# NVIDIA/DALI

Hardware: NVIDIA H100
Metric: images/sec decode+resize+CMN (batch 256, 1080p JPEG) (higher is better)
Workload: dtype u8

## Files before the change

### dali_b200/csrc/jpeg.cu

```cuda
#include "common.cuh"
#include <algorithm>
#include <cstring>
#include <map>
#include <thread>

namespace dalib200 {

constexpr int kDcLutBits = 9, kAcLutBits = 11;
constexpr int kDcLutSize = 1 << kDcLutBits, kAcLutSize = 1 << kAcLutBits;
constexpr int kLutWords = 2 * kDcLutSize + 2 * kAcLutSize;
constexpr int kSyncThreads = 256;
constexpr int kChunkBytes = 4096;
constexpr int kMaxBlocksPerMcu = 10;
constexpr int kMaxLog2Sub = 10;

constexpr int kLongLut = 512;
struct HuffSlow {
  int32_t maxcode[18];
  int32_t valoff[18];
  uint8_t vals[256];
  int32_t long_base, long_n;
  uint16_t long_lut[kLongLut];
};

struct TableSet {
  uint32_t lut[kLutWords];
  uint16_t lut16[kLutWords];
  HuffSlow slow[4];
};
__host__ __device__ inline int LutOffset(int t) { return t < 2 ? t * kDcLutSize : 2 * kDcLutSize + (t - 2) * kAcLutSize; }

struct QuantSet { uint16_t q[4][64]; };

enum JpegColor : int32_t {
  kColorGray = 0,
// ... 193 lines not shown
#pragma unroll
      for (int w = 0; w < 8; w++) { if (w < (int)wid) woff += wsum[w][r]; tot += wsum[w][r]; }
      uint32_t pos = head + total + (uint32_t)(woff + incl[r] - cw.nk[r]);
      const uint32_t i = (uint32_t)r * 1024u + threadIdx.x * 4u;
#pragma unroll
      for (int k = 0; k < 4; k++)
        if (i + k < len && !((cw.dm[r] >> (8 * k)) & 1u)) ob[pos++] = (uint8_t)(cw.w[r] >> (8 * k));
      total += (uint32_t)tot;
    }
    __syncthreads();
    const uint32_t nwords = (head + total + 3u) >> 2, tailb = (head + total) & 3u;
    uint32_t *cw32 = reinterpret_cast<uint32_t *>(clean) + (out_base >> 2);
    for (uint32_t wd = threadIdx.x; wd < nwords; wd += blockDim.x) {
      const uint32_t v = obuf[wd];
      const bool full = (wd > 0 || head == 0) && (wd + 1 < nwords || tailb == 0);
      if (full) {
        cw32[wd] = __byte_perm(v, 0u, 0x0123);
      } else {
        const uint32_t lo = wd == 0 ? head : 0u, hi = (wd + 1 == nwords && tailb) ? tailb : 4u;
        for (uint32_t b = lo; b < hi; b++) reinterpret_cast<uint8_t *>(cw32 + wd)[3u - b] = (uint8_t)(v >> (8 * b));
      }
    }
    if (c0 + kChunkBytes >= u.raw_len) {
      const uint32_t e0 = out_base + total, e1 = u.clean_off + ((u.raw_len + 32u + 15u) & ~15u);
      for (uint32_t q = e0 + threadIdx.x; q < e1; q += blockDim.x) clean[(q & ~3u) | (3u - (q & 3u))] = 0;
    }
    __syncthreads();
  }
}

struct SmemSrc {
  uint32_t base; int lsw;
  __device__ __forceinline__ uint32_t load(uint32_t g) const { return lds_u32(base + ((g ^ ((g >> lsw) & 31u)) << 2)); }
};
struct SmemLut { uint32_t base; __device__ __forceinline__ uint32_t load(uint32_t i) const { return lds_u32(base + (i << 2)); } };
struct GlobalLut { const uint32_t *p; __device__ __forceinline__ uint32_t load(uint32_t i) const { return __ldg(p + i); } };
template <int STRIDE> struct SmemTbl { uint32_t base; __device__ __forceinline__ uint32_t load(int c) const { return lds_u32(base + (uint32_t)c * (STRIDE * 4u)); } };
struct GlobalSrc {
  const uint32_t *w;
  __device__ __forceinline__ uint32_t load(uint32_t g) const { return __ldg(w + g); }
};

template <class Src>
struct BitWindow {
  uint32_t hi, lo, g;
  int avail;
  __device__ __forceinline__ void init(const Src &s, uint32_t word, uint32_t sh) {
    const uint32_t w0 = s.load(word), w1 = s.load(word + 1);
    hi = __funnelshift_l(w1, w0, sh);
    lo = w1 << sh;
    avail = 64 - (int)sh;
    g = word + 2;
  }
  __device__ __forceinline__ void consume(const Src &s, uint32_t e) {
    hi = __funnelshift_l(lo, hi, e);
    lo = __funnelshift_l(0u, lo, e);
    avail -= (int)(e & 31u);
    const uint32_t w = s.load(g);
    const bool need = avail < 32;
    const uint32_t a = (uint32_t)avail & 31u;
    hi |= (need ? w : 0u) >> a;
    lo = need ? (w << ((32u - a) & 31u)) : lo;
    avail += need ? 32 : 0;
    g += need ? 1u : 0u;
  }
};

constexpr uint64_t kStateMask = (1ull << 42) - 1;
constexpr uint32_t kMaxChainLen = 4095;
__device__ __forceinline__ uint64_t pack_state(uint32_t p, int c, int z, uint32_t cnt = 0, uint32_t t = 0) {
  return (uint64_t)p | ((uint64_t)(uint32_t)c << 32) | ((uint64_t)(uint32_t)z << 36) | ((uint64_t)min(cnt, 1023u) << 42) | ((uint64_t)t << 52);
}
__device__ __forceinline__ uint32_t state_count(uint64_t s) { return (uint32_t)(s >> 42) & 1023u; }

__device__ __forceinline__ uint32_t make_entry(uint32_t len, uint32_t sym, bool is_dc) {
  const uint32_t s = sym & 15u, r = sym >> 4;
  const uint32_t adv = is_dc ? 1u : (s == 0 ? (r == 15u ? 16u : 64u) : r + 1u);
  return (len + s) | (s << 8) | (len << 12) | (adv << 20);
}

__device__ __forceinline__ uint32_t make_entry16(uint32_t len, uint32_t sym, bool is_dc) {
  const uint32_t s = sym & 15u, r = sym >> 4;
  const uint32_t adv = is_dc ? 1u : (s == 0 ? (r == 15u ? 16u : 64u) : r + 1u);
  return (len + s) | (s << 5) | (adv << 9);
}

__device__ __noinline__ uint32_t slow_lookup(const HuffSlow *__restrict__ slow, uint32_t toff, uint32_t hi, bool is_dc) {
  const int tbl = toff < 2u * kDcLutSize ? (int)(toff / kDcLutSize) : 2 + (int)((toff - 2u * kDcLutSize) / kAcLutSize);
  const HuffSlow *sl = slow + tbl;
  const int32_t code16 = (int32_t)(hi >> 16);
  if (sl->long_n > 0) {
    const int idx = min(max(code16 - sl->long_base, 0), sl->long_n - 1);
    const uint32_t e = sl->long_lut[idx];
    return e ? e : 16u;
  }
  uint32_t len = (is_dc ? kDcLutBits : kAcLutBits) + 1;
  while (len <= 16 && code16 >= sl->maxcode[len]) len++;
  uint32_t sym = 0;
  if (len > 16) len = 16;
  else sym = sl->vals[(sl->valoff[len] + (code16 >> (16 - len))) & 0xFF];
  return len | (sym << 8);
}
__device__ __forceinline__ uint32_t slow_symbol(const HuffSlow *__restrict__ slow, uint32_t toff, uint32_t hi, bool is_dc) {
  const uint32_t ls = slow_lookup(slow, toff, hi, is_dc);
  return make_entry(ls & 0xFFu, ls >> 8, is_dc);
}
__device__ __forceinline__ uint32_t slow_symbol16(const HuffSlow *__restrict__ slow, uint32_t toff, uint32_t hi, bool is_dc) {
  const uint32_t ls = slow_lookup(slow, toff, hi, is_dc);
  return make_entry16(ls & 0xFFu, ls >> 8, is_dc);
}

template <class Src, class Lut, class Tbl>
__device__ __forceinline__ void decode_span(const Src &src, BitWindow<Src> &win, const Lut &lut, const HuffSlow *__restrict__ slow,
                                            const Tbl &tbl, int bpm, uint32_t &pos, uint32_t end, int &c, int &z, uint32_t &nb) {
  uint32_t tb12 = tbl.load(c);
  while (pos < end) {
    const uint32_t e_ac = lut.load((tb12 >> 16) + (win.hi >> (32 - kAcLutBits)));
    const bool is_dc = z == 0;
    uint32_t e = e_ac;
    if (is_dc) e = lut.load((tb12 & 0xFFFFu) + (win.hi >> (32 - kDcLutBits)));
    if (__builtin_expect(e == 0, 0)) e = slow_symbol(slow, is_dc ? (tb12 & 0xFFFFu) : (tb12 >> 16), win.hi, is_dc);
    const uint32_t tb = e & 31u, adv = e >> 20;
    win.consume(src, e);
    pos += tb;
    z += (int)adv;
    const bool endb = z >= 64;
    const int c1 = c + 1 == bpm ? 0 : c + 1;
    nb += endb ? 1u : 0u;
    c = endb ? c1 : c;
    z = endb ? 0 : z;
    if (endb) tb12 = tbl.load(c);
  }
}

__device__ __forceinline__ int find_unit_by_subseq(const JpegUnit *u, int ub, int ue, int j) {
  int lo = ub, hi = ue - 1;
  while (lo < hi) {
    int mid = (lo + hi + 1) >> 1;
    if (u[mid].first_subseq <= j) lo = mid; else hi = mid - 1;
  }
  return lo;
}

struct HuffCtx {
  const JpegImage *images; int nimages;
  const int32_t *block_image;
// ... 99 lines not shown
}

__device__ __forceinline__ void push_chain(const HuffCtx &cx, int list, uint32_t pos, int c, int z, uint32_t t, int64_t g, int img) {
  const uint32_t k = atomicAdd(&cx.chain_count[list], 1u);
  cx.chains[list][k] = make_uint4(pos, (uint32_t)c | ((uint32_t)z << 8) | (t << 16), (uint32_t)g, (uint32_t)img);
}

__global__ void __launch_bounds__(kSyncThreads) huff_sync_intra_kernel(HuffCtx cx) {
  extern __shared__ __align__(16) uint32_t hsm[];
  const SyncSmem sm = carve_sync_smem(hsm, cx.log2_sub);
  const int img_i = cx.block_image[blockIdx.x];
  const JpegImage &im = cx.images[img_i];
  const SubGeom sg = sync_block_prologue(cx, im, sm);
  const HuffSlow *slow = sm.slow;
  const int lsw = cx.log2_sub - 5;
  const SmemSrc src{smem_u32(sm.sw), lsw};
  const SmemLut lut{smem_u32(sm.lut)};
  const SmemTbl<1> tbl{smem_u32(sm.tbl)};
  BitWindow<SmemSrc> win;
  uint32_t pos = sg.jl << cx.log2_sub, nb = 0;
  int c = 0, z = 0;
  if (sg.valid) {
    win.init(src, (uint32_t)threadIdx.x << lsw, 0);
    decode_span(src, win, lut, slow, tbl, im.bpm, pos, sm.col_end[threadIdx.x], c, z, nb);
    sm.exitst[threadIdx.x] = pack_state(pos, c, z);
    sm.cnt[threadIdx.x] = nb;
  }
  __syncthreads();
  if (sm.col_cont[threadIdx.x]) {
    if (threadIdx.x + 1 == kSyncThreads) {
      push_chain(cx, 0, pos, c, z, 1u, sg.g + 1, img_i);
    } else {
      const uint32_t x = threadIdx.x + 1;
      nb = 0;
      decode_span(src, win, lut, slow, tbl, im.bpm, pos, sm.col_end[x], c, z, nb);
      const uint64_t ns = pack_state(pos, c, z);
      const bool same = sm.exitst[x] == ns;
      sm.exitst[x] = ns; sm.cnt[x] = nb;
      if (!same && sm.col_cont[x]) push_chain(cx, 0, pos, c, z, 2u, sg.g + 2, img_i);
    }
  }
  __syncthreads();
  if (sg.valid) {
    const uint32_t t = threadIdx.x > 0 && sm.col_cont[threadIdx.x - 1] ? 1u : 0u;
    cx.s_state[sg.g] = sm.exitst[threadIdx.x] | ((uint64_t)min(sm.cnt[threadIdx.x], 1023u) << 42) | ((uint64_t)t << 52);
  }
}

constexpr int kTailThreads = 256;
constexpr int kTailColWords = 36;
struct ColSrc {
  uint32_t base;
  __device__ __forceinline__ uint32_t load(uint32_t g) const { return lds_u32(base + g * (kTailThreads * 4u)); }
};

__device__ __forceinline__ void walk_chain(const HuffCtx &cx, const uint4 rec, int out_list, int max_visits, const uint32_t *s_lut,
                                           const HuffSlow *s_slow, int s_table_set, uint32_t *col, uint32_t *tblcol) {
  const int img_i = (int)rec.w;
  const JpegImage &im = cx.images[img_i];
  int64_t g = rec.z;
  const int j = (int)(g - im.subseq_begin);
  const int ui = im.unit_end - im.unit_begin == 1 ? im.unit_begin : find_unit_by_subseq(cx.units, im.unit_begin, im.unit_end, j);
  const JpegUnit &u = cx.units[ui];
  const uint32_t clean_bits = cx.unit_clean_len[ui] * 8u;
  const uint32_t nsub_eff = (clean_bits + (1u << cx.log2_sub) - 1) >> cx.log2_sub;
  uint32_t jl = (uint32_t)(j - u.first_subseq);
#pragma unroll
  for (int b = 0; b < kMaxBlocksPerMcu; b++) tblcol[b * kTailThreads] = tbl_word(im, b);
  const bool shared_tables = im.table_set == s_table_set;
  uint32_t pos = rec.x, t = rec.y >> 16;
  int c = (int)(rec.y & 0xFF), z = (int)((rec.y >> 8) & 0xFF);
  const int sub_words = 1 << (cx.log2_sub - 5);
  for (int visit = 0;;) {
    uint32_t nb = 0;
    const uint32_t end = min((jl + 1) << cx.log2_sub, clean_bits);
    if (shared_tables && sub_words + 4 <= kTailColWords) {
      const uint4 *p4 = reinterpret_cast<const uint4 *>(cx.clean + u.clean_off + ((size_t)jl << (cx.log2_sub - 3)));
      for (int q = 0; q < sub_words / 4 + 1; q++) {
        const uint4 v = __ldg(p4 + q);
        col[(4 * q + 0) * kTailThreads] = v.x; col[(4 * q + 1) * kTailThreads] = v.y;
        col[(4 * q + 2) * kTailThreads] = v.z; col[(4 * q + 3) * kTailThreads] = v.w;
      }
      const ColSrc src{smem_u32(col)};
      const uint32_t rel = pos - (jl << cx.log2_sub);
      BitWindow<ColSrc> win;
      win.init(src, rel >> 5, rel & 31u);
      decode_span(src, win, SmemLut{smem_u32(s_lut)}, s_slow, SmemTbl<kTailThreads>{smem_u32(tblcol)}, im.bpm, pos, end, c, z, nb);
    } else {
      const GlobalSrc src{reinterpret_cast<const uint32_t *>(cx.clean + u.clean_off)};
      BitWindow<GlobalSrc> win;
      win.init(src, pos >> 5, pos & 31u);
      decode_span(src, win, GlobalLut{cx.tables[im.table_set].lut}, cx.tables[im.table_set].slow, SmemTbl<kTailThreads>{smem_u32(tblcol)},
                  im.bpm, pos, end, c, z, nb);
    }
    const uint64_t ns = pack_state(pos, c, z, nb, t);
    const uint64_t old = atomicMax(reinterpret_cast<unsigned long long *>(cx.s_state + g), (unsigned long long)ns);
    if ((uint32_t)(old >> 52) >= t) break;
    if (((old ^ ns) & kStateMask) == 0) break;
    if (jl + 1 >= nsub_eff || t >= kMaxChainLen) break;
    g++; jl++; t++;
    if (++visit >= max_visits) { push_chain(cx, out_list, pos, c, z, t, g, img_i); break; }
  }
}

__global__ void __launch_bounds__(kTailThreads) huff_sync_walk_kernel(HuffCtx cx, int in_list, int out_list, int max_visits) {
  extern __shared__ __align__(16) uint32_t tsm[];
  const uint32_t n = cx.chain_count[in_list];
  if (blockIdx.x * blockDim.x >= n) return;
  uint32_t *s_lut = tsm;
  HuffSlow *s_slow = reinterpret_cast<HuffSlow *>(s_lut + kLutWords);
  uint32_t *col = reinterpret_cast<uint32_t *>(s_slow + 4) + threadIdx.x;
  uint32_t *tblcol = reinterpret_cast<uint32_t *>(s_slow + 4) + kTailColWords * kTailThreads + threadIdx.x;
  const int s_table_set = cx.images[0].table_set;
  {
    const uint4 *src = reinterpret_cast<const uint4 *>(cx.tables[s_table_set].lut);
// ... 23 lines not shown
    __syncthreads();
    for (uint32_t base = 0; base < nsub_eff; base += blockDim.x) {
      const uint32_t i = base + threadIdx.x;
      const uint32_t v = i < nsub_eff ? state_count(cx.s_state[g0 + i]) : 0u;
      uint32_t incl = v;
      for (int o = 1; o < 32; o <<= 1) { uint32_t x = __shfl_up_sync(0xffffffffu, incl, o); if ((threadIdx.x & 31) >= o) incl += x; }
      if ((threadIdx.x & 31) == 31) warp_tot[threadIdx.x >> 5] = incl;
      __syncthreads();
      uint32_t woff = 0, tot = 0;
      for (int w = 0; w < (int)(blockDim.x >> 5); w++) { if (w < (int)(threadIdx.x >> 5)) woff += warp_tot[w]; tot += warp_tot[w]; }
      if (i < nsub_eff) cx.s_n[g0 + i] = carry + woff + incl - v;
      __syncthreads();
      if (threadIdx.x == 0) carry += tot;
      __syncthreads();
    }
    if (threadIdx.x == 0) {
      if ((int64_t)carry * 64 < u.nslots) cx.status[blockIdx.x] = 1;
      cx.unit_nblk[ui] = (uint32_t)min((int64_t)carry, u.nslots >> 6);
    }
  }
}

constexpr int kWriteThreads = 384;
struct WriteSmem {
  uint16_t *lut; uint32_t *sw, *tbl, *blkbuf; uint8_t *zig; HuffSlow *slow; const uint8_t **colptr;
};
__host__ __device__ inline size_t write_sw_words(int log2_sub) { return (size_t)(kWriteThreads + look_ahead_cols(log2_sub)) << (log2_sub - 5); }
__host__ __device__ inline size_t write_smem_bytes(int log2_sub) {
  return kLutWords * 2 + write_sw_words(log2_sub) * 4 + 16 * 4  + 64  + (size_t)kWriteThreads * 128;
}
__device__ __forceinline__ WriteSmem carve_write_smem(uint32_t *base, int log2_sub) {
  WriteSmem s;
  s.lut = reinterpret_cast<uint16_t *>(base);
  s.sw = base + kLutWords / 2;
  s.tbl = s.sw + write_sw_words(log2_sub);
  s.zig = reinterpret_cast<uint8_t *>(s.tbl + 16);
  s.slow = nullptr;
  s.blkbuf = reinterpret_cast<uint32_t *>(s.zig + 64);
  s.colptr = reinterpret_cast<const uint8_t **>(s.blkbuf);
  return s;
}

__global__ void __launch_bounds__(kWriteThreads) huff_write_kernel(HuffCtx cx) {
  extern __shared__ __align__(16) uint32_t hsm[];
  const WriteSmem sm = carve_write_smem(hsm, cx.log2_sub);
  const JpegImage &im = cx.images[cx.wblock_image[blockIdx.x]];
  const int lsw = cx.log2_sub - 5;
  {
    const uint4 *src = reinterpret_cast<const uint4 *>(cx.tables[im.table_set].lut16);
    uint4 *dst = reinterpret_cast<uint4 *>(sm.lut);
    for (int i = threadIdx.x; i < kLutWords * 2 / 16; i += blockDim.x) dst[i] = __ldg(src + i);
    if (threadIdx.x < kMaxBlocksPerMcu) sm.tbl[threadIdx.x] = tbl_word(im, threadIdx.x);
    if (threadIdx.x < 64) sm.zig[threadIdx.x] = c_zigzag[threadIdx.x];
  }
  SubGeom sg;
  {
    const int j = (blockIdx.x - im.wblock_begin) * kWriteThreads + threadIdx.x;
    sg.valid = j < im.nsub;
    sg.ui = 0; sg.jl = 0; sg.nsub_eff = 0; sg.clean_bits = 0;
    sg.g = (int64_t)im.subseq_begin + j;
    const uint8_t *ptr = nullptr;
    if (sg.valid) {
      sg.ui = im.unit_end - im.unit_begin == 1 ? im.unit_begin : find_unit_by_subseq(cx.units, im.unit_begin, im.unit_end, j);
      const JpegUnit &u = cx.units[sg.ui];
      sg.clean_bits = cx.unit_clean_len[sg.ui] * 8u;
      sg.nsub_eff = (sg.clean_bits + (1u << cx.log2_sub) - 1) >> cx.log2_sub;
      sg.jl = (uint32_t)(j - u.first_subseq);
      sg.valid = sg.jl < sg.nsub_eff;
      if (sg.valid) ptr = cx.clean + u.clean_off + ((size_t)sg.jl << (cx.log2_sub - 3));
    }
    sm.colptr[threadIdx.x] = ptr;
    const int la_cols = look_ahead_cols(cx.log2_sub);
    if (threadIdx.x == kWriteThreads - 1)
      for (int q = 1; q <= la_cols; q++) sm.colptr[kWriteThreads - 1 + q] = ptr ? ptr + ((size_t)q << (cx.log2_sub - 3)) : nullptr;
    __syncthreads();
    const int cpc = 1 << (cx.log2_sub - 7);
    for (int ch = threadIdx.x; ch < (kWriteThreads + la_cols) * cpc; ch += blockDim.x) {
      const int col = ch / cpc, o = ch - col * cpc;
      const uint8_t *p = sm.colptr[col];
      if (p) {
        const uint4 v = __ldg(reinterpret_cast<const uint4 *>(p) + o);
        const uint32_t g = ((uint32_t)col << lsw) + 4u * o, x = (uint32_t)col & 31u;
        sm.sw[(g + 0) ^ x] = v.x; sm.sw[(g + 1) ^ x] = v.y; sm.sw[(g + 2) ^ x] = v.z; sm.sw[(g + 3) ^ x] = v.w;
      }
    }
    __syncthreads();
  }
  const HuffSlow *slow = cx.tables[im.table_set].slow;
  const SmemSrc src{smem_u32(sm.sw), lsw};
  const uint32_t lane = threadIdx.x & 31u;
  const uint32_t a_lut = smem_u32(sm.lut), a_tbl = smem_u32(sm.tbl), a_zig = smem_u32(sm.zig);
  const uint32_t a_wbuf = smem_u32(sm.blkbuf) + (threadIdx.x & ~31u) * 128u;
  const uint32_t a_mybuf = a_wbuf + lane * 128u;
#pragma unroll
  for (int j = 0; j < 32; j++) sts_u32(a_mybuf + 4u * j, 0u);
  __syncwarp();
  uint32_t pos = 0, nb = 0, end = 0, hard_end = 0, blk0 = 0, blk_limit = 0;
  int c = 0, z = 0;
  bool active = sg.valid;
  if (active) {
    const JpegUnit &u = cx.units[sg.ui];
    if (sg.jl > 0) {
      const uint64_t prev = cx.s_state[sg.g - 1];
      pos = (uint32_t)prev; c = (int)((prev >> 32) & 15u); z = (int)((prev >> 36) & 63u);
    }
    end = min((sg.jl + 1) << cx.log2_sub, sg.clean_bits);
    hard_end = sg.clean_bits;
    const uint32_t ublk = (uint32_t)(u.slot_base >> 6);
    blk0 = ublk + cx.s_n[sg.g];
    blk_limit = ublk + (uint32_t)(u.nslots >> 6);
    active = pos < end && blk0 < blk_limit;
  }
  bool own = z == 0;
  BitWindow<SmemSrc> win;
  {
    const uint32_t rel = active ? pos - (sg.jl << cx.log2_sub) : 0u;
    win.init(src, ((uint32_t)threadIdx.x << lsw) + (rel >> 5), rel & 31u);
  }
  int16_t *coef = cx.coef + im.coef_off;
  int16_t *dcv = cx.dc + im.coef_off / 64;
  const int bpm = im.bpm;
  uint32_t tb12 = lds_u32(a_tbl + 4u * c);
  while (__any_sync(0xffffffffu, active)) {
    bool flush = false;
    const uint32_t blk = blk0 + nb;
    if (active) {
      const uint32_t e_ac = lds_u16(a_lut + 2u * ((tb12 >> 16) + (win.hi >> (32 - kAcLutBits))));
      const bool is_dc = z == 0;
      uint32_t e = e_ac;
      if (is_dc) e = lds_u16(a_lut + 2u * ((tb12 & 0xFFFFu) + (win.hi >> (32 - kDcLutBits))));
      if (__builtin_expect(e == 0, 0)) e = slow_symbol16(slow, is_dc ? (tb12 & 0xFFFFu) : (tb12 >> 16), win.hi, is_dc);
      const uint32_t tb = e & 31u, adv = e >> 9, s = (e >> 5) & 15u;
      {
        const uint32_t len = tb - s;
        const uint32_t bits = (uint32_t)(((uint64_t)(win.hi << len)) >> (32u - s));
        const int v = (int)bits - ((s == 0 || ((bits >> (s - 1u)) & 1u)) ? 0 : (int)((1u << s) - 1u));
        if (own) {
          if (is_dc) {
            dcv[blk] = (int16_t)v;
          } else if (s) {
            const uint32_t nat = lds_u8(a_zig + min((uint32_t)z + adv - 1u, 63u));
            sts_u16(a_mybuf + 4u * ((nat >> 1) ^ lane) + 2u * (nat & 1u), (uint32_t)v);
          }
        }
      }
      win.consume(src, e);
      pos += tb;
      z += (int)adv;
      const bool endb = z >= 64;
      const int c1 = c + 1 == bpm ? 0 : c + 1;
      flush = endb && own;
      nb += endb ? 1u : 0u;
      own = own || endb;
      c = endb ? c1 : c;
      z = endb ? 0 : z;
      if (endb) tb12 = lds_u32(a_tbl + 4u * c);
      active = blk0 + nb < blk_limit && (pos < end || (z != 0 && pos < hard_end));
    }
    uint32_t m = __ballot_sync(0xffffffffu, flush);
    while (m) {
      const uint32_t L = __ffs(m) - 1u;
      m &= m - 1u;
      const uint32_t fb = __shfl_sync(0xffffffffu, blk, L);
      const uint32_t a_src = a_wbuf + L * 128u + 4u * (lane ^ L);
      const uint32_t w = lds_u32(a_src);
      sts_u32(a_src, 0u);
      reinterpret_cast<uint32_t *>(coef + (size_t)fb * 64)[lane] = w;
    }
    __syncwarp();
// ... 826 lines not shown
  std::vector<int> post_sample;
  std::vector<size_t> post_off;
  std::vector<int32_t> out_shape;
  std::vector<uint8_t> planes_only;
  std::vector<JpegGeo> geo;
  std::vector<int64_t> first_work;
  std::vector<int64_t> first_fused;
  int64_t total_work = 0, total_fused = 0, total_post_px = 0;
  size_t post_bytes = 0;
  uint8_t *d_post = nullptr; size_t d_post_cap = 0;
  JpegPost *d_posts = nullptr; size_t d_posts_cap = 0;
  std::vector<ParsedJpeg> parsed;
  std::vector<JpegImage> images;
  std::vector<JpegUnit> units;
  std::vector<TableSet> tables;
  std::vector<QuantSet> quants;
  std::vector<int64_t> first_quad, first_item;
  std::vector<int32_t> block_image;
  std::vector<int32_t> wblock_image;
  std::vector<const uint8_t *> src_ptr;
  bool source_stable = false;
  int last_upload_direct = 0;
  std::vector<size_t> stage_off;
  size_t raw_bytes = 0, clean_bytes = 0;
  uint32_t nchunks = 0;
  int64_t total_subseq = 0, total_coefs = 0, total_plane_bytes = 0, total_quads = 0, total_items = 0;
  int total_blocks_sync = 0, total_blocks_write = 0;
  int log2_sub = 10;
  uint8_t *h_stage = nullptr; size_t h_stage_cap = 0;
  uint8_t *d_stage = nullptr; size_t d_stage_cap = 0;
  size_t desc_bytes = 0, off_images = 0, off_units = 0, off_tables = 0, off_quants = 0, off_quads = 0, off_items = 0, off_work = 0, off_fused = 0, off_blkimg = 0, off_wblkimg = 0, off_raw = 0;
  uint8_t *d_clean = nullptr; size_t d_clean_cap = 0;
  uint32_t *d_chunk = nullptr; size_t d_chunk_cap = 0;
  uint32_t *d_unit_len = nullptr; size_t d_unit_cap = 0;
  uint64_t *d_state = nullptr; uint32_t *d_n = nullptr; size_t d_sub_cap = 0;
  uint4 *d_chain1 = nullptr, *d_chain2 = nullptr, *d_chain3 = nullptr;
  size_t d_chain1_cap = 0, d_chain2_cap = 0, d_chain3_cap = 0;
  uint32_t *d_chain_count = nullptr; size_t d_chain_count_cap = 0;
  int walk_max_grid = 0;
  int16_t *d_coef = nullptr; size_t d_coef_cap = 0;
  int16_t *d_dc = nullptr; size_t d_dc_cap = 0;
  uint8_t *d_planes = nullptr; size_t d_planes_cap = 0;
  int32_t *d_status = nullptr; size_t d_status_cap = 0;
  uint32_t *d_unit_nblk = nullptr; size_t d_unit_nblk_cap = 0;
  int32_t *h_status = nullptr; size_t h_status_cap = 0;
  cudaEvent_t uploaded = nullptr, img_uploaded = nullptr;
  uint8_t *h_images = nullptr; size_t h_images_cap = 0;
// ... 176 lines not shown
  p->dtype = prm->dtype; p->adjust_orientation = prm->adjust_orientation != 0;
  p->posts.clear(); p->post_sample.clear(); p->post_off.clear();
  p->out_shape.assign((size_t)3 * n, 0);
  p->planes_only.assign(n, 0);
  p->geo.assign(n, JpegGeo());
  p->first_work.assign(n, 0);
  p->first_fused.assign(n, 0);

  p->parsed.assign(n, ParsedJpeg());
  p->images.assign(n, JpegImage());
  p->units.clear(); p->tables.clear(); p->quants.clear(); p->src_ptr.clear(); p->block_image.clear(); p->wblock_image.clear();
  p->first_quad.assign(n, 0);
  p->first_item.assign(n, 0);
  p->prog_images.clear(); p->prog_scans.clear(); p->prog_huff.clear(); p->prog_wave_begin.clear(); p->prog_first_blk.clear();
  p->prog_total_blocks = 0;
  std::map<std::string, int> table_cache, quant_cache, prog_table_cache;
  size_t raw = 0, clean = 0;
  uint32_t chunks = 0;
  int64_t subseq = 0, coefs = 0, planes = 0;
  int sync_blocks = 0, write_blocks = 0;
  size_t total_len = 0;
  for (int i = 0; i < n; i++) total_len += lengths[i];
  int log2_bytes = kMaxLog2Sub - 3;
  if (const char *ev = getenv("DALIB200_JPEG_SUBSEQ_BYTES")) { int v = atoi(ev); log2_bytes = v >= 256 ? 8 : v >= 128 ? 7 : v >= 64 ? 6 : 5; }
  while (log2_bytes > 5 && (total_len >> log2_bytes) < 200000) log2_bytes--;
  p->log2_sub = log2_bytes + 3;
  const size_t sub_bytes = (size_t)1 << log2_bytes;
  for (int i = 0; i < n; i++) {
    ParsedJpeg &j = p->parsed[i];
    DB_CHECK_ARG(streams[i] && lengths[i] > 0, "decoders.image: sample %d is empty", i);
    int rc = ParseHeaders(streams[i], lengths[i], j, true);
    if (rc) { std::string m = dalib200GetLastError(); SetLastError("decoders.image: sample %d: %s", i, m.c_str()); return rc; }
    auto unsupported = [&](const char *what) { SetLastError("decoders.image: sample %d: %s", i, what); return DALIB200_ERROR_UNSUPPORTED; };
    const bool prog = j.progressive || (j.ncomp > 1 && j.scan_ncomp != j.ncomp);
    if (prog) {
      j.scan_ncomp = j.ncomp;
      for (int c = 0; c < j.ncomp; c++) { j.scan_comp[c] = c; j.td[c] = j.ta[c] = 0; }
    }
    if ((int64_t)j.width * j.height >= (1ll << 31)) return unsupported("images of 2^31 pixels or more are not supported");
    if (j.precision != 8) return unsupported("only 8-bit baseline JPEG is supported");
    if (j.ncomp != 1 && j.ncomp != 3 && j.ncomp != 4) return unsupported("only 1-, 3- or 4-component JPEG is supported");
    if (j.scan_ncomp != j.ncomp) return unsupported("multi-scan (non-interleaved) baseline JPEG is not supported yet");
    if (j.ncomp == 3)
      for (int c = 1; c < j.ncomp; c++)
        if (j.hs[c] != 1 || j.vs[c] != 1) return unsupported("chroma sampling factors other than 1x1 are not supported");
    if (j.ncomp == 4)
      for (int c = 0; c < j.ncomp; c++)
        if (j.hmax % j.hs[c] || j.vmax % j.vs[c]) return unsupported("non-integral component sampling ratios are not supported");
// ... 57 lines not shown
    }
    const uint8_t *d = streams[i];
    size_t sb = j.scan_begin, se = lengths[i];
    if (se >= sb + 2 && d[se - 2] == 0xFF && d[se - 1] == 0xD9) se -= 2;
    j.scan_end = se;
    const int64_t nmcu = (int64_t)im.mcux * im.mcuy;
    im.unit_begin = (int)p->units.size();
    im.subseq_begin = (int)subseq;
    im.block_begin = sync_blocks;
    im.wblock_begin = write_blocks;
    int32_t local_sub = 0;
    auto add_unit = [&](size_t b, size_t e, int64_t mcu0, int64_t mcus) {
      JpegUnit u;
      memset(&u, 0, sizeof(u));
      u.raw_off = (uint32_t)(raw + (b - sb));
      u.raw_len = (uint32_t)(e - b);
      u.clean_off = (uint32_t)clean;
      u.first_chunk = chunks;
      u.image = i;
      u.first_subseq = local_sub;
      u.nsub_max = (int32_t)((u.raw_len + sub_bytes - 1) / sub_bytes);
      u.slot_base = mcu0 * bpm * 64;
      u.nslots = mcus * bpm * 64;
      clean += Align(u.raw_len + 32, 16);
      chunks += (u.raw_len + kChunkBytes - 1) / kChunkBytes;
      local_sub += u.nsub_max;
      p->units.push_back(u);
    };
    if (prog) {
      dalib200::ProgImage pim;
      memset(&pim, 0, sizeof(pim));
      std::string perr;
      const size_t first_new = p->prog_scans.size();
      rc = dalib200::PlanProgressive(d, lengths[i], sb, (int)p->prog_images.size(), &pim, p->prog_scans, p->prog_huff, prog_table_cache, &perr);
      if (rc) { SetLastError("decoders.image: sample %d: %s", i, perr.c_str()); return rc; }
      for (size_t k = first_new; k < p->prog_scans.size(); k++)
        if ((size_t)p->prog_scans[k].data_off + p->prog_scans[k].data_len > se - sb) {
          auto &sc = p->prog_scans[k];
          sc.data_len = sc.data_off >= se - sb ? 0 : (uint32_t)(se - sb - sc.data_off);
        }
      if (pim.ncomp != im.ncomp || pim.mcux != im.mcux || pim.mcuy != im.mcuy || pim.bpm != bpm) {
        SetLastError("decoders.image: sample %d: internal error (progressive frame layout)", i); return DALIB200_ERROR_INTERNAL;
      }
      pim.sample = i;
      pim.raw_off = (int64_t)raw;
      pim.coef_off = coefs;
      p->prog_first_blk.push_back(p->prog_total_blocks);
// ... 76 lines not shown
    const bool planes_only = rois && rois[i].planes_only;
    if (planes_only && !ge.planar_ok) {
      SetLastError("decoders.image: sample %d: planes_only needs a 3-component 4:2:0 YCbCr stream without orientation, RGB u8 output", i);
      return DALIB200_ERROR_UNSUPPORTED;
    }
    p->planes_only[i] = planes_only;
    {
      const int mw = 8 * j.hmax, mh = 8 * j.vmax, ex = 2 * j.hmax, ey = 2 * j.vmax;
      const int mx0 = std::max(0, im.win_x0 - ex) / mw, mx1 = std::min(im.mcux - 1, (im.win_x0 + im.win_w - 1 + ex) / mw);
      const int my0 = std::max(0, im.win_y0 - ey) / mh, my1 = std::min(im.mcuy - 1, (im.win_y0 + im.win_h - 1 + ey) / mh);
      im.mcu_x0 = mx0; im.mcu_y0 = my0; im.mcu_nx = mx1 - mx0 + 1; im.mcu_ny = my1 - my0 + 1;
    }
  }
  BuildWorkLists(p);
  if (!p->prog_scans.empty()) {
    std::stable_sort(p->prog_scans.begin(), p->prog_scans.end(), [](const dalib200::ProgScan &a, const dalib200::ProgScan &b) { return a.wave < b.wave; });
    const int nw = p->prog_scans.back().wave + 1;
    p->prog_wave_begin.assign(nw + 1, 0);
    for (const auto &sc : p->prog_scans) p->prog_wave_begin[sc.wave + 1]++;
    for (int w = 0; w < nw; w++) p->prog_wave_begin[w + 1] += p->prog_wave_begin[w];
  }
  DB_CHECK_ARG(raw < (1ull << 32) && clean < (1ull << 32), "decoders.image: batch of encoded data exceeds 4 GiB");
  p->raw_bytes = raw; p->clean_bytes = clean; p->nchunks = chunks;
  p->total_subseq = subseq; p->total_coefs = coefs; p->total_plane_bytes = planes;
  p->total_blocks_sync = sync_blocks; p->total_blocks_write = write_blocks;
  size_t off = 0;
  p->off_images = off; off += Align(sizeof(JpegImage) * n, 16);
  p->off_units = off; off += Align(sizeof(JpegUnit) * p->units.size(), 16);
  p->off_tables = off; off += Align(sizeof(TableSet) * p->tables.size(), 16);
  p->off_quants = off; off += Align(sizeof(QuantSet) * p->quants.size(), 16);
  p->off_quads = off; off += Align(sizeof(int64_t) * n, 16);
  p->off_items = off; off += Align(sizeof(int64_t) * n, 16);
  p->off_work = off; off += Align(sizeof(int64_t) * n, 16);
  p->off_fused = off; off += Align(sizeof(int64_t) * n, 16);
  p->off_blkimg = off; off += Align(sizeof(int32_t) * p->block_image.size(), 16);
  p->off_wblkimg = off; off += Align(sizeof(int32_t) * p->wblock_image.size(), 16);
  p->off_raw = off;
  p->desc_bytes = off;
  const size_t total = off + raw + 64;
  if (p->pending) { DB_CUDA(cudaEventSynchronize(p->uploaded)); p->pending = false; }
  if (total > p->h_stage_cap) {
    if (p->h_stage) cudaFreeHost(p->h_stage);
    p->h_stage = nullptr; p->h_stage_cap = 0;
    size_t ncap = total + total / 4;
    DB_CUDA(cudaMallocHost(reinterpret_cast<void **>(&p->h_stage), ncap));
    p->h_stage_cap = ncap;
// ... 147 lines not shown
    std::vector<std::thread> th;
    if (p->raw_bytes >= (1u << 20)) for (int t = 0; t < nthreads; t++) th.emplace_back(work);
    else work();
    cudaError_t err = cudaSuccess;
    for (int g = 0; g < G; g++) {
      while (done[g].load(std::memory_order_acquire) < group_cnt[g]) std::this_thread::yield();
      const size_t b0 = group_begin[g], b1 = g + 1 < G ? group_begin[g + 1] : p->raw_bytes;
      if (err == cudaSuccess && b1 > b0)
        err = cudaMemcpyAsync(p->d_stage + p->off_raw + b0, p->h_stage + p->off_raw + b0, b1 - b0, cudaMemcpyHostToDevice, stream);
    }
    for (auto &t : th) t.join();
    DB_CUDA(err);
  }
  DB_CUDA(cudaEventRecord(p->uploaded, stream));
  p->pending = true;
  return DALIB200_SUCCESS;
} DB_API_CATCH

int dalib200JpegLaunch(dalib200JpegPlan *p, void *const *out_ptrs, dalib200Stream_t stream) try {
  DB_CHECK_ARG(p && p->staged && out_ptrs, "JpegLaunch: call JpegPlanSetup / JpegUpload first");
  if (p->n == 0) return DALIB200_SUCCESS;
  DB_CHECK_ARG(p->d_stage && p->d_stage_cap >= p->desc_bytes + p->raw_bytes, "JpegLaunch: JpegUpload has not been called for this batch");
  int rc;
  if ((rc = GrowDevice(p->d_clean, p->d_clean_cap, p->clean_bytes + 1024))) return rc;
  if ((rc = GrowDevice(p->d_chunk, p->d_chunk_cap, (size_t)p->nchunks + 1))) return rc;
  if ((rc = GrowDevice(p->d_unit_len, p->d_unit_cap, p->units.size() + 1))) return rc;
  {
    size_t cap2 = p->d_sub_cap;
    if ((rc = GrowDevice(p->d_state, p->d_sub_cap, (size_t)p->total_subseq + 1))) return rc;
    if ((rc = GrowDevice(p->d_n, cap2, (size_t)p->total_subseq + 1))) return rc;
  }
  if ((rc = GrowDevice(p->d_chain1, p->d_chain1_cap, (size_t)p->total_subseq + 1))) return rc;
  if ((rc = GrowDevice(p->d_chain2, p->d_chain2_cap, (size_t)p->total_subseq + 1))) return rc;
  if ((rc = GrowDevice(p->d_chain3, p->d_chain3_cap, (size_t)p->total_subseq + 1))) return rc;
  if ((rc = GrowDevice(p->d_chain_count, p->d_chain_count_cap, (size_t)8))) return rc;
  if ((rc = GrowDevice(p->d_coef, p->d_coef_cap, (size_t)p->total_coefs + 64))) return rc;
  if ((rc = GrowDevice(p->d_dc, p->d_dc_cap, (size_t)p->total_coefs / 64 + 64))) return rc;
  if ((rc = GrowDevice(p->d_planes, p->d_planes_cap, (size_t)p->total_plane_bytes + 64))) return rc;
  if ((rc = GrowDevice(p->d_status, p->d_status_cap, (size_t)p->n + 1))) return rc;
  if ((rc = GrowDevice(p->d_unit_nblk, p->d_unit_nblk_cap, p->units.size() + 1))) return rc;
  if (!p->posts.empty()) {
    if ((rc = GrowDevice(p->d_post, p->d_post_cap, p->post_bytes + 256))) return rc;
    if ((rc = GrowDevice(p->d_posts, p->d_posts_cap, p->posts.size()))) return rc;
  }
  {
    if (p->img_pending) { DB_CUDA(cudaEventSynchronize(p->img_uploaded)); p->img_pending = false; }
    const size_t img_bytes = Align(sizeof(JpegImage) * p->n, 16);
// ... 56 lines not shown
    a.d_huff = reinterpret_cast<const ProgHuff *>(p->prog_arena.dev + o_huff);
    a.d_first_blk = reinterpret_cast<const int64_t *>(p->prog_arena.dev + o_blk);
    a.total_blocks = p->prog_total_blocks;
    a.wave_begin = &p->prog_wave_begin; a.h_images = &p->prog_images;
    a.d_raw = d_raw; a.d_coef = p->d_coef; a.d_dc = p->d_dc; a.d_status = p->d_status;
    if ((rc = LaunchProgressive(a, ps))) return rc;
    DB_CUDA(cudaEventRecord(p->prog_join, ps));
  }
  const bool any_units = nunits > 0 && p->nchunks > 0 && p->total_blocks_sync > 0;
  if (any_units) {
    const int grid = (int)std::min<uint32_t>(p->nchunks, (uint32_t)sms * 16);
    { ProfScope ps_("jpeg_unstuff_count", s); unstuff_count_kernel<<<grid, 256, 0, s>>>(d_raw, d_units, nunits, p->nchunks, p->d_chunk); }
    { ProfScope ps_("jpeg_unstuff_scan", s); unstuff_scan_kernel<<<(nunits + 7) / 8, 256, 0, s>>>(d_units, nunits, p->d_chunk, p->d_unit_len); }
    { ProfScope ps_("jpeg_unstuff_scatter", s); unstuff_scatter_kernel<<<grid, 256, 0, s>>>(d_raw, d_units, nunits, p->nchunks, p->d_chunk, p->d_clean); }
    CountLaunch(3);
  }
  HuffCtx cx;
  cx.images = d_images; cx.nimages = p->n; cx.block_image = reinterpret_cast<const int32_t *>(p->d_stage + p->off_blkimg);
  cx.wblock_image = reinterpret_cast<const int32_t *>(p->d_stage + p->off_wblkimg);
  cx.units = d_units; cx.unit_clean_len = p->d_unit_len; cx.tables = d_tables;
  cx.clean = p->d_clean; cx.s_state = p->d_state; cx.s_n = p->d_n; cx.coef = p->d_coef; cx.dc = p->d_dc; cx.log2_sub = p->log2_sub;
  cx.status = p->d_status; cx.unit_nblk = p->d_unit_nblk;
  cx.chains[0] = p->d_chain1; cx.chains[1] = p->d_chain2; cx.chains[2] = p->d_chain3; cx.chain_count = p->d_chain_count;
  const size_t hsmem = sync_smem_bytes(p->log2_sub, false), wsmem = write_smem_bytes(p->log2_sub);
  const size_t walk_smem = kLutWords * 4 + 4 * sizeof(HuffSlow) + (size_t)(kTailColWords + kMaxBlocksPerMcu) * kTailThreads * 4;
  if (!p->smem_opted) {
    DB_CUDA(cudaFuncSetAttribute(huff_sync_intra_kernel, cudaFuncAttributeMaxDynamicSharedMemorySize, (int)sync_smem_bytes(kMaxLog2Sub, false)));
    DB_CUDA(cudaFuncSetAttribute(huff_write_kernel, cudaFuncAttributeMaxDynamicSharedMemorySize, (int)write_smem_bytes(kMaxLog2Sub)));
    DB_CUDA(cudaFuncSetAttribute(huff_sync_walk_kernel, cudaFuncAttributeMaxDynamicSharedMemorySize, (int)walk_smem));
    int per_sm = 0;
    DB_CUDA(cudaOccupancyMaxActiveBlocksPerMultiprocessor(&per_sm, huff_sync_walk_kernel, kTailThreads, walk_smem));
    p->walk_max_grid = std::max(1, per_sm) * sms * 4;
    p->smem_opted = true;
  }
  if (any_units) { ProfScope ps_("jpeg_huff_sync_intra", s); huff_sync_intra_kernel<<<p->total_blocks_sync, kSyncThreads, hsmem, s>>>(cx); }
  if (any_units) {
    auto walk_grid = [&](double frac) {
      const int64_t want = (int64_t)(p->total_subseq * frac) / kTailThreads + p->total_blocks_sync / kTailThreads + 1;
      return (int)std::max<int64_t>(1, std::min<int64_t>(p->walk_max_grid, want));
    };
    { ProfScope ps_("jpeg_huff_sync_walk1", s); huff_sync_walk_kernel<<<walk_grid(0.40), kTailThreads, walk_smem, s>>>(cx, 0, 1, 1); }
    { ProfScope ps_("jpeg_huff_sync_walk2", s); huff_sync_walk_kernel<<<walk_grid(0.14), kTailThreads, walk_smem, s>>>(cx, 1, 2, 1); }
    { ProfScope ps_("jpeg_huff_sync_walk3", s); huff_sync_walk_kernel<<<walk_grid(0.06), kTailThreads, walk_smem, s>>>(cx, 2, 0, 1 << 30); }
    CountLaunch(2);
  }
  { ProfScope ps_("jpeg_huff_scan", s); huff_scan_kernel<<<p->n, 1024, 0, s>>>(cx); }
  CountLaunch();
  if (any_units && p->total_blocks_write > 0) { ProfScope ps_("jpeg_huff_write", s); huff_write_kernel<<<p->total_blocks_write, kWriteThreads, wsmem, s>>>(cx); }
  if (!p->prog_images.empty()) DB_CUDA(cudaStreamWaitEvent(s, p->prog_join, 0));
  { ProfScope ps_("jpeg_dc_scan", s); dc_scan_kernel<<<p->n, 1024, 0, s>>>(d_images, p->d_dc); }
  { ProfScope ps_("jpeg_truncation_fixup", s); truncation_fixup_kernel<<<p->n, 256, 0, s>>>(cx); }
// ... 39 lines not shown
```

Before: 38460.

## Stream Huffman write-kernel bits from global memory instead of staging in shared memory

The Huffman write kernel no longer stages each thread's subsequence plus look-ahead columns into shared memory. Each thread now reads its bitstream directly from global memory through a register window, refilled with predicated 16-byte non-coherent loads on alternate iterations. This drops the staging copy and two block barriers and shrinks shared memory, which allows a launch bound of 3 CTAs per SM. The clean buffer is padded for over-read and the subsequence-size env override now skips auto-shrinking. In exchange it adds register pressure and makes decoding depend on global-load latency being hidden.

```diff
diff --git a/dali_b200/csrc/jpeg.cu b/dali_b200/csrc/jpeg.cu
--- a/dali_b200/csrc/jpeg.cu
+++ b/dali_b200/csrc/jpeg.cu
@@ -11,6 +11,7 @@
 constexpr int kLutWords = 2 * kDcLutSize + 2 * kAcLutSize;
 constexpr int kSyncThreads = 256;
 constexpr int kChunkBytes = 4096;
+constexpr uint32_t kCleanPad = 32;
 constexpr int kMaxBlocksPerMcu = 10;
 constexpr int kMaxLog2Sub = 10;
 
@@ -250,7 +251,7 @@
       }
     }
     if (c0 + kChunkBytes >= u.raw_len) {
-      const uint32_t e0 = out_base + total, e1 = u.clean_off + ((u.raw_len + 32u + 15u) & ~15u);
+      const uint32_t e0 = out_base + total, e1 = u.clean_off + ((u.raw_len + kCleanPad + 15u) & ~15u);
       for (uint32_t q = e0 + threadIdx.x; q < e1; q += blockDim.x) clean[(q & ~3u) | (3u - (q & 3u))] = 0;
     }
     __syncthreads();
@@ -271,16 +272,18 @@
 
 template <class Src>
 struct BitWindow {
+  Src s;
   uint32_t hi, lo, g;
   int avail;
-  __device__ __forceinline__ void init(const Src &s, uint32_t word, uint32_t sh) {
+  __device__ __forceinline__ void init(const Src &src, uint32_t word, uint32_t sh) {
+    s = src;
     const uint32_t w0 = s.load(word), w1 = s.load(word + 1);
     hi = __funnelshift_l(w1, w0, sh);
     lo = w1 << sh;
     avail = 64 - (int)sh;
     g = word + 2;
   }
-  __device__ __forceinline__ void consume(const Src &s, uint32_t e) {
+  __device__ __forceinline__ void consume(uint32_t e) {
     hi = __funnelshift_l(lo, hi, e);
     lo = __funnelshift_l(0u, lo, e);
     avail -= (int)(e & 31u);
@@ -294,6 +297,57 @@
   }
 };
 
+constexpr uint32_t kStreamReadBehind = 60;
+__device__ __forceinline__ void ldg_stream(bool pred, uint4 &v, const uint4 *p) {
+  asm volatile("{\n\t.reg .pred q;\n\tsetp.ne.u32 q, %5, 0;\n\t@q ld.global.nc.L2::128B.v4.u32 {%0, %1, %2, %3}, [%4];\n\t}"
+               : "+r"(v.x), "+r"(v.y), "+r"(v.z), "+r"(v.w) : "l"(p), "r"((uint32_t)pred));
+}
+struct StreamWindow {
+  uint32_t hi, lo;
+  int avail;
+  uint32_t left;
+  uint32_t c0, c1, c2, c3, c4;
+  uint4 nxt;
+  const uint4 *p;
+  __device__ __forceinline__ void clear() { left = 5; }
+  __device__ __forceinline__ void init(const uint8_t *unit, uint32_t pos) {
+    const uint4 *q = reinterpret_cast<const uint4 *>(unit) + (pos >> 7);
+    const uint4 a = __ldg(q);
+    nxt = __ldg(q + 1);
+    p = q + 2;
+    hi = a.x; lo = a.y; avail = 64;
+    c0 = a.z; c1 = a.w; c2 = c3 = c4 = 0; left = 2;
+    for (uint32_t d = pos & 127u; d;) {
+      const uint32_t e = min(d, 31u);
+      consume(e);
+      top_up();
+      d -= e;
+    }
+  }
+  __device__ __forceinline__ void consume(uint32_t e) {
+    hi = __funnelshift_l(lo, hi, e);
+    lo = __funnelshift_l(0u, lo, e);
+    avail -= (int)(e & 31u);
+    const bool need = avail < 32;
+    const uint32_t a = (uint32_t)avail & 31u;
+    hi |= (need ? c0 : 0u) >> a;
+    lo = need ? (c0 << ((32u - a) & 31u)) : lo;
+    avail += need ? 32 : 0;
+    c0 = need ? c1 : c0; c1 = need ? c2 : c1; c2 = need ? c3 : c2; c3 = need ? c4 : c3;
+    left -= need ? 1u : 0u;
+  }
+  __device__ __forceinline__ void top_up() {
+    const bool take = left <= 1;
+    if (take) {
+      const bool one = left != 0;
+      c0 = one ? c0 : nxt.x; c1 = one ? nxt.x : nxt.y; c2 = one ? nxt.y : nxt.z; c3 = one ? nxt.z : nxt.w; c4 = nxt.w;
+      left += 4;
+    }
+    ldg_stream(take, nxt, p);
+    p += take ? 1 : 0;
+  }
+};
+
 constexpr uint64_t kStateMask = (1ull << 42) - 1;
 constexpr uint32_t kMaxChainLen = 4095;
 __device__ __forceinline__ uint64_t pack_state(uint32_t p, int c, int z, uint32_t cnt = 0, uint32_t t = 0) {
@@ -338,8 +392,8 @@
   return make_entry16(ls & 0xFFu, ls >> 8, is_dc);
 }
 
-template <class Src, class Lut, class Tbl>
-__device__ __forceinline__ void decode_span(const Src &src, BitWindow<Src> &win, const Lut &lut, const HuffSlow *__restrict__ slow,
+template <class Win, class Lut, class Tbl>
+__device__ __forceinline__ void decode_span(Win &win, const Lut &lut, const HuffSlow *__restrict__ slow,
                                             const Tbl &tbl, int bpm, uint32_t &pos, uint32_t end, int &c, int &z, uint32_t &nb) {
   uint32_t tb12 = tbl.load(c);
   while (pos < end) {
@@ -349,7 +403,7 @@
     if (is_dc) e = lut.load((tb12 & 0xFFFFu) + (win.hi >> (32 - kDcLutBits)));
     if (__builtin_expect(e == 0, 0)) e = slow_symbol(slow, is_dc ? (tb12 & 0xFFFFu) : (tb12 >> 16), win.hi, is_dc);
     const uint32_t tb = e & 31u, adv = e >> 20;
-    win.consume(src, e);
+    win.consume(e);
     pos += tb;
     z += (int)adv;
     const bool endb = z >= 64;
@@ -495,7 +549,7 @@
   int c = 0, z = 0;
   if (sg.valid) {
     win.init(src, (uint32_t)threadIdx.x << lsw, 0);
-    decode_span(src, win, lut, slow, tbl, im.bpm, pos, sm.col_end[threadIdx.x], c, z, nb);
+    decode_span(win, lut, slow, tbl, im.bpm, pos, sm.col_end[threadIdx.x], c, z, nb);
     sm.exitst[threadIdx.x] = pack_state(pos, c, z);
     sm.cnt[threadIdx.x] = nb;
   }
@@ -506,7 +560,7 @@
     } else {
       const uint32_t x = threadIdx.x + 1;
       nb = 0;
-      decode_span(src, win, lut, slow, tbl, im.bpm, pos, sm.col_end[x], c, z, nb);
+      decode_span(win, lut, slow, tbl, im.bpm, pos, sm.col_end[x], c, z, nb);
       const uint64_t ns = pack_state(pos, c, z);
       const bool same = sm.exitst[x] == ns;
       sm.exitst[x] = ns; sm.cnt[x] = nb;
@@ -522,6 +576,10 @@
 
 constexpr int kTailThreads = 256;
 constexpr int kTailColWords = 36;
+__host__ __device__ inline uint32_t clean_read_behind(int log2_sub) {
+  const uint32_t sub = 1u << (log2_sub - 3), staged = sub + (uint32_t)look_ahead_cols(log2_sub) * sub;
+  return staged > kStreamReadBehind ? staged : kStreamReadBehind;
+}
 struct ColSrc {
   uint32_t base;
   __device__ __forceinline__ uint32_t load(uint32_t g) const { return lds_u32(base + g * (kTailThreads * 4u)); }
@@ -558,12 +616,12 @@
       const uint32_t rel = pos - (jl << cx.log2_sub);
       BitWindow<ColSrc> win;
       win.init(src, rel >> 5, rel & 31u);
-      decode_span(src, win, SmemLut{smem_u32(s_lut)}, s_slow, SmemTbl<kTailThreads>{smem_u32(tblcol)}, im.bpm, pos, end, c, z, nb);
+      decode_span(win, SmemLut{smem_u32(s_lut)}, s_slow, SmemTbl<kTailThreads>{smem_u32(tblcol)}, im.bpm, pos, end, c, z, nb);
     } else {
       const GlobalSrc src{reinterpret_cast<const uint32_t *>(cx.clean + u.clean_off)};
       BitWindow<GlobalSrc> win;
       win.init(src, pos >> 5, pos & 31u);
-      decode_span(src, win, GlobalLut{cx.tables[im.table_set].lut}, cx.tables[im.table_set].slow, SmemTbl<kTailThreads>{smem_u32(tblcol)},
+      decode_span(win, GlobalLut{cx.tables[im.table_set].lut}, cx.tables[im.table_set].slow, SmemTbl<kTailThreads>{smem_u32(tblcol)},
                   im.bpm, pos, end, c, z, nb);
     }
     const uint64_t ns = pack_state(pos, c, z, nb, t);
@@ -633,30 +691,24 @@
 }
 
 constexpr int kWriteThreads = 384;
+constexpr int kWriteCtasPerSm = 3;
 struct WriteSmem {
-  uint16_t *lut; uint32_t *sw, *tbl, *blkbuf; uint8_t *zig; HuffSlow *slow; const uint8_t **colptr;
+  uint16_t *lut; uint32_t *tbl, *blkbuf; uint8_t *zig;
 };
-__host__ __device__ inline size_t write_sw_words(int log2_sub) { return (size_t)(kWriteThreads + look_ahead_cols(log2_sub)) << (log2_sub - 5); }
-__host__ __device__ inline size_t write_smem_bytes(int log2_sub) {
-  return kLutWords * 2 + write_sw_words(log2_sub) * 4 + 16 * 4  + 64  + (size_t)kWriteThreads * 128;
-}
-__device__ __forceinline__ WriteSmem carve_write_smem(uint32_t *base, int log2_sub) {
+__host__ __device__ inline size_t write_smem_bytes() { return kLutWords * 2 + 16 * 4  + 64  + (size_t)kWriteThreads * 128; }
+__device__ __forceinline__ WriteSmem carve_write_smem(uint32_t *base) {
   WriteSmem s;
   s.lut = reinterpret_cast<uint16_t *>(base);
-  s.sw = base + kLutWords / 2;
-  s.tbl = s.sw + write_sw_words(log2_sub);
+  s.tbl = base + kLutWords / 2;
   s.zig = reinterpret_cast<uint8_t *>(s.tbl + 16);
-  s.slow = nullptr;
   s.blkbuf = reinterpret_cast<uint32_t *>(s.zig + 64);
-  s.colptr = reinterpret_cast<const uint8_t **>(s.blkbuf);
   return s;
 }
 
-__global__ void __launch_bounds__(kWriteThreads) huff_write_kernel(HuffCtx cx) {
+__global__ void __launch_bounds__(kWriteThreads, kWriteCtasPerSm) huff_write_kernel(HuffCtx cx) {
   extern __shared__ __align__(16) uint32_t hsm[];
-  const WriteSmem sm = carve_write_smem(hsm, cx.log2_sub);
+  const WriteSmem sm = carve_write_smem(hsm);
   const JpegImage &im = cx.images[cx.wblock_image[blockIdx.x]];
-  const int lsw = cx.log2_sub - 5;
   {
     const uint4 *src = reinterpret_cast<const uint4 *>(cx.tables[im.table_set].lut16);
     uint4 *dst = reinterpret_cast<uint4 *>(sm.lut);
@@ -670,7 +722,6 @@
     sg.valid = j < im.nsub;
     sg.ui = 0; sg.jl = 0; sg.nsub_eff = 0; sg.clean_bits = 0;
     sg.g = (int64_t)im.subseq_begin + j;
-    const uint8_t *ptr = nullptr;
     if (sg.valid) {
       sg.ui = im.unit_end - im.unit_begin == 1 ? im.unit_begin : find_unit_by_subseq(cx.units, im.unit_begin, im.unit_end, j);
       const JpegUnit &u = cx.units[sg.ui];
@@ -678,27 +729,9 @@
       sg.nsub_eff = (sg.clean_bits + (1u << cx.log2_sub) - 1) >> cx.log2_sub;
       sg.jl = (uint32_t)(j - u.first_subseq);
       sg.valid = sg.jl < sg.nsub_eff;
-      if (sg.valid) ptr = cx.clean + u.clean_off + ((size_t)sg.jl << (cx.log2_sub - 3));
-    }
-    sm.colptr[threadIdx.x] = ptr;
-    const int la_cols = look_ahead_cols(cx.log2_sub);
-    if (threadIdx.x == kWriteThreads - 1)
-      for (int q = 1; q <= la_cols; q++) sm.colptr[kWriteThreads - 1 + q] = ptr ? ptr + ((size_t)q << (cx.log2_sub - 3)) : nullptr;
-    __syncthreads();
-    const int cpc = 1 << (cx.log2_sub - 7);
-    for (int ch = threadIdx.x; ch < (kWriteThreads + la_cols) * cpc; ch += blockDim.x) {
-      const int col = ch / cpc, o = ch - col * cpc;
-      const uint8_t *p = sm.colptr[col];
-      if (p) {
-        const uint4 v = __ldg(reinterpret_cast<const uint4 *>(p) + o);
-        const uint32_t g = ((uint32_t)col << lsw) + 4u * o, x = (uint32_t)col & 31u;
-        sm.sw[(g + 0) ^ x] = v.x; sm.sw[(g + 1) ^ x] = v.y; sm.sw[(g + 2) ^ x] = v.z; sm.sw[(g + 3) ^ x] = v.w;
-      }
-    }
-    __syncthreads();
+    }
   }
   const HuffSlow *slow = cx.tables[im.table_set].slow;
-  const SmemSrc src{smem_u32(sm.sw), lsw};
   const uint32_t lane = threadIdx.x & 31u;
   const uint32_t a_lut = smem_u32(sm.lut), a_tbl = smem_u32(sm.tbl), a_zig = smem_u32(sm.zig);
   const uint32_t a_wbuf = smem_u32(sm.blkbuf) + (threadIdx.x & ~31u) * 128u;
@@ -723,18 +756,18 @@
     active = pos < end && blk0 < blk_limit;
   }
   bool own = z == 0;
-  BitWindow<SmemSrc> win;
-  {
-    const uint32_t rel = active ? pos - (sg.jl << cx.log2_sub) : 0u;
-    win.init(src, ((uint32_t)threadIdx.x << lsw) + (rel >> 5), rel & 31u);
-  }
+  StreamWindow win;
+  win.clear();
+  if (active) win.init(cx.clean + cx.units[sg.ui].clean_off, pos);
+  __syncthreads();
   int16_t *coef = cx.coef + im.coef_off;
   int16_t *dcv = cx.dc + im.coef_off / 64;
   const int bpm = im.bpm;
   uint32_t tb12 = lds_u32(a_tbl + 4u * c);
-  while (__any_sync(0xffffffffu, active)) {
+  for (uint32_t it = 1; __any_sync(0xffffffffu, active); it++) {
     bool flush = false;
     const uint32_t blk = blk0 + nb;
+    if (it & 1u) win.top_up();
     if (active) {
       const uint32_t e_ac = lds_u16(a_lut + 2u * ((tb12 >> 16) + (win.hi >> (32 - kAcLutBits))));
       const bool is_dc = z == 0;
@@ -755,7 +788,7 @@
           }
         }
       }
-      win.consume(src, e);
+      win.consume(e);
       pos += tb;
       z += (int)adv;
       const bool endb = z >= 64;
@@ -1628,7 +1661,7 @@
   bool source_stable = false;
   int last_upload_direct = 0;
   std::vector<size_t> stage_off;
-  size_t raw_bytes = 0, clean_bytes = 0;
+  size_t raw_bytes = 0, clean_bytes = 0, clean_alloc = 0;
   uint32_t nchunks = 0;
   int64_t total_subseq = 0, total_coefs = 0, total_plane_bytes = 0, total_quads = 0, total_items = 0;
   int total_blocks_sync = 0, total_blocks_write = 0;
@@ -1851,8 +1884,12 @@
   size_t total_len = 0;
   for (int i = 0; i < n; i++) total_len += lengths[i];
   int log2_bytes = kMaxLog2Sub - 3;
-  if (const char *ev = getenv("DALIB200_JPEG_SUBSEQ_BYTES")) { int v = atoi(ev); log2_bytes = v >= 256 ? 8 : v >= 128 ? 7 : v >= 64 ? 6 : 5; }
-  while (log2_bytes > 5 && (total_len >> log2_bytes) < 200000) log2_bytes--;
+  if (const char *ev = getenv("DALIB200_JPEG_SUBSEQ_BYTES")) {
+    const int v = atoi(ev);
+    log2_bytes = v >= 128 ? 7 : v >= 64 ? 6 : 5;
+  } else {
+    while (log2_bytes > 5 && (total_len >> log2_bytes) < 200000) log2_bytes--;
+  }
   p->log2_sub = log2_bytes + 3;
   const size_t sub_bytes = (size_t)1 << log2_bytes;
   for (int i = 0; i < n; i++) {
@@ -1956,7 +1993,7 @@
       u.nsub_max = (int32_t)((u.raw_len + sub_bytes - 1) / sub_bytes);
       u.slot_base = mcu0 * bpm * 64;
       u.nslots = mcus * bpm * 64;
-      clean += Align(u.raw_len + 32, 16);
+      clean += Align(u.raw_len + kCleanPad, 16);
       chunks += (u.raw_len + kChunkBytes - 1) / kChunkBytes;
       local_sub += u.nsub_max;
       p->units.push_back(u);
@@ -2079,6 +2116,11 @@
   }
   DB_CHECK_ARG(raw < (1ull << 32) && clean < (1ull << 32), "decoders.image: batch of encoded data exceeds 4 GiB");
   p->raw_bytes = raw; p->clean_bytes = clean; p->nchunks = chunks;
+  p->clean_alloc = clean + (clean_read_behind(p->log2_sub) - kCleanPad);
+  for (const JpegUnit &u : p->units)
+    if ((size_t)u.clean_off + u.raw_len + clean_read_behind(p->log2_sub) > p->clean_alloc) {
+      SetLastError("decoders.image: internal error (clean stream read bound)"); return DALIB200_ERROR_INTERNAL;
+    }
   p->total_subseq = subseq; p->total_coefs = coefs; p->total_plane_bytes = planes;
   p->total_blocks_sync = sync_blocks; p->total_blocks_write = write_blocks;
   size_t off = 0;
@@ -2272,7 +2314,7 @@
   if (p->n == 0) return DALIB200_SUCCESS;
   DB_CHECK_ARG(p->d_stage && p->d_stage_cap >= p->desc_bytes + p->raw_bytes, "JpegLaunch: JpegUpload has not been called for this batch");
   int rc;
-  if ((rc = GrowDevice(p->d_clean, p->d_clean_cap, p->clean_bytes + 1024))) return rc;
+  if ((rc = GrowDevice(p->d_clean, p->d_clean_cap, p->clean_alloc))) return rc;
   if ((rc = GrowDevice(p->d_chunk, p->d_chunk_cap, (size_t)p->nchunks + 1))) return rc;
   if ((rc = GrowDevice(p->d_unit_len, p->d_unit_cap, p->units.size() + 1))) return rc;
   {
@@ -2375,11 +2417,11 @@
   cx.clean = p->d_clean; cx.s_state = p->d_state; cx.s_n = p->d_n; cx.coef = p->d_coef; cx.dc = p->d_dc; cx.log2_sub = p->log2_sub;
   cx.status = p->d_status; cx.unit_nblk = p->d_unit_nblk;
   cx.chains[0] = p->d_chain1; cx.chains[1] = p->d_chain2; cx.chains[2] = p->d_chain3; cx.chain_count = p->d_chain_count;
-  const size_t hsmem = sync_smem_bytes(p->log2_sub, false), wsmem = write_smem_bytes(p->log2_sub);
+  const size_t hsmem = sync_smem_bytes(p->log2_sub, false), wsmem = write_smem_bytes();
   const size_t walk_smem = kLutWords * 4 + 4 * sizeof(HuffSlow) + (size_t)(kTailColWords + kMaxBlocksPerMcu) * kTailThreads * 4;
   if (!p->smem_opted) {
     DB_CUDA(cudaFuncSetAttribute(huff_sync_intra_kernel, cudaFuncAttributeMaxDynamicSharedMemorySize, (int)sync_smem_bytes(kMaxLog2Sub, false)));
-    DB_CUDA(cudaFuncSetAttribute(huff_write_kernel, cudaFuncAttributeMaxDynamicSharedMemorySize, (int)write_smem_bytes(kMaxLog2Sub)));
+    DB_CUDA(cudaFuncSetAttribute(huff_write_kernel, cudaFuncAttributeMaxDynamicSharedMemorySize, (int)wsmem));
     DB_CUDA(cudaFuncSetAttribute(huff_sync_walk_kernel, cudaFuncAttributeMaxDynamicSharedMemorySize, (int)walk_smem));
     int per_sm = 0;
     DB_CUDA(cudaOccupancyMaxActiveBlocksPerMultiprocessor(&per_sm, huff_sync_walk_kernel, kTailThreads, walk_smem));
```

After: 39720 (median of 6 runs). 1.03x the previous value.
